# aanna0701/face-recognition-pytorch

Measured on AMD Instinct MI355X. Metric: train imgs/sec IR-50-layout ResNet50 + ArcFace/PartialFC head, 112x112, higher is better.
Workload: dtype bf16

## Files before the change

### face-recognition-pytorch_amd/frhip/csrc/igemm_nt.h

```cpp
#pragma once
#include "common.h"

namespace frhip {

struct NtGeom {
    int H, W, C;
    int Ho, Wo;
    int R, S, stride, pad;
    int mode;
    int M, Nout, Ktot;
    int ksteps, ksteps_per_split;
    uint32_t a_bytes, b_bytes;
    int par_a, par_b, hc, wc, par_r0, par_s0;
};

struct OutMap {
    int hc, wc, ho, wo, a, b;
    __device__ __forceinline__ long long row(int m) const {
        if (wc == 0) return m;
        const int per = hc * wc;
        const int img = m / per, rem = m - img * per;
        const int i = rem / wc, j = rem - i * wc;
        return ((long long)img * ho + 2 * i + a) * wo + 2 * j + b;
    }
};

constexpr int NT_ROWB = 128;

struct EpiBnRed {
    const void* y;
    const float* mean;
    const float* invstd;
    const float* mscale;
    const float* mshift;
    int res_h, res_w;
    OutMap map;
    const float* bias;
    void* act;
    int gelu_bwd;
    const float* aff_scale;
    const float* aff_shift;
    int aff_relu;
    const float* rowkeep;
    int rows_per;
    float keep_scale;
};

template <typename T, int WM, int WN, int MT = 4>
struct NtTile {
    static constexpr int WAVES = WM * WN, THREADS = 64 * WAVES;
    static constexpr int WROWS = MT * 16;
    static constexpr int BM = WM * WROWS, BN = WN * 64;
    static constexpr int BKE = NT_ROWB / (int)sizeof(T);
    static constexpr int STAGE_BYTES = (BM + BN) * NT_ROWB;
    static constexpr int A_PIECES = BM / 8 / WAVES, B_PIECES = BN / 8 / WAVES;
    static_assert(A_PIECES * 8 * WAVES == BM && B_PIECES * 8 * WAVES == BN, "tile rows must split evenly over the waves");
    template <typename TS> static constexpr int stage_pitch() { return 64 * (int)sizeof(TS) + 16; }
    template <typename TS> static constexpr int lds_bytes() {
        return (2 * STAGE_BYTES > WAVES * WROWS * stage_pitch<TS>()) ? 2 * STAGE_BYTES : WAVES * WROWS * stage_pitch<TS>();
    }
};

template <int NPIECE>
struct RowSet {
    int pixbase[NPIECE];
    int hb[NPIECE], wb[NPIECE];
};

template <typename T, int WM, int WN, int MT = 4>
struct NtMainloop {
    typedef NtTile<T, WM, WN, MT> Tile;
    typedef typename Mma<T>::Frag Frag;
    static constexpr int BM = Tile::BM, BN = Tile::BN, BKE = Tile::BKE;

    f32x4_t acc[4][MT];

    __device__ __forceinline__ void run(const NtGeom& g, const void* __restrict__ a_ptr,
                                        const void* __restrict__ b_ptr, char* smem,
                                        int mtile, int ntile, int ks_begin, int ks_end) {
        const int lane = lane_id();
        const int wave = wave_id();
        const int wm = wave / WN, wn = wave % WN;
#pragma unroll
        for (int i = 0; i < 4; ++i)
#pragma unroll
            for (int j = 0; j < MT; ++j) acc[i][j] = f32x4_t{0.f, 0.f, 0.f, 0.f};
        if (ks_begin >= ks_end) return;

        const __amdgpu_buffer_rsrc_t ra = make_rsrc(a_ptr, g.a_bytes);
        const __amdgpu_buffer_rsrc_t rb = make_rsrc(b_ptr, g.b_bytes);

        const int sub = lane >> 3;
        const uint32_t chunk_bytes = (uint32_t)(((lane & 7) ^ sub) * 16);
        RowSet<Tile::A_PIECES> ar;
        const int rowlen = g.par_a >= 0 ? g.wc : g.Wo;
        const int HoWo = g.par_a >= 0 ? g.hc * g.wc : g.Ho * g.Wo;
#pragma unroll
        for (int j = 0; j < Tile::A_PIECES; ++j) {
            const int row = (wave * Tile::A_PIECES + j) * 8 + sub;
            const int m = mtile * BM + row;
            if (m < g.M) {
                const int n = m / HoWo, rem = m - n * HoWo;
                int ho = rem / rowlen, wo = rem - ho * rowlen;
                if (g.par_a >= 0) { ho = 2 * ho + g.par_a; wo = 2 * wo + g.par_b; }
                ar.pixbase[j] = n * g.H * g.W;
                if (g.mode == 0) { ar.hb[j] = ho * g.stride - g.pad; ar.wb[j] = wo * g.stride - g.pad; }
                else             { ar.hb[j] = ho + g.pad;            ar.wb[j] = wo + g.pad; }
            } else {
                ar.pixbase[j] = -1; ar.hb[j] = 0; ar.wb[j] = 0;
            }
        }
        uint32_t brow_off[Tile::B_PIECES];
#pragma unroll
        for (int j = 0; j < Tile::B_PIECES; ++j) {
            const int row = (wave * Tile::B_PIECES + j) * 8 + sub;
            const int n = ntile * BN + row;
            brow_off[j] = (n < g.Nout) ? (uint32_t)n * (uint32_t)g.Ktot * (uint32_t)sizeof(T) + chunk_bytes
                                       : OOB_OFFSET;
        }

        const int cchunks = g.C / BKE;
        int tap = ks_begin / cchunks;
        int c0 = (ks_begin - tap * cchunks) * BKE;
        int fr = tap / g.S, fs = tap - fr * g.S;
        const int tstep = g.par_a >= 0 ? 2 : 1, fs0 = g.par_a >= 0 ? g.par_s0 : 0;
        if (g.par_a >= 0) {
            const int ns = (g.S - g.par_s0 + 1) >> 1;
            const int ir = tap / ns, is = tap - ir * ns;
            fr = g.par_r0 + 2 * ir; fs = g.par_s0 + 2 * is;
            tap = fr * g.S + fs;
        }

        auto stage = [&](int buf) {
            char* sa = smem + buf * Tile::STAGE_BYTES;
            char* sb = sa + BM * NT_ROWB;
#pragma unroll
            for (int j = 0; j < Tile::A_PIECES; ++j) {
                int hi, wi; bool ok = ar.pixbase[j] >= 0;
                if (g.mode == 0) {
                    hi = ar.hb[j] + fr; wi = ar.wb[j] + fs;
                } else {
                    const int th = ar.hb[j] - fr, tw = ar.wb[j] - fs;
                    ok = ok && th >= 0 && tw >= 0;
                    if (g.stride == 2) { ok = ok && !((th | tw) & 1); hi = th >> 1; wi = tw >> 1; }
                    else { hi = th; wi = tw; }
                }
                ok = ok && (unsigned)hi < (unsigned)g.H && (unsigned)wi < (unsigned)g.W;
                const uint32_t off = ok ? (uint32_t)((ar.pixbase[j] + hi * g.W + wi) * g.C + c0) * (uint32_t)sizeof(T) + chunk_bytes
                                        : OOB_OFFSET;
                glds16(ra, sa + (wave * Tile::A_PIECES + j) * 1024, off);
            }
            const uint32_t kb = (uint32_t)(tap * g.C + c0) * (uint32_t)sizeof(T);
#pragma unroll
            for (int j = 0; j < Tile::B_PIECES; ++j) {
                const uint32_t off = brow_off[j] == OOB_OFFSET ? OOB_OFFSET : brow_off[j] + kb;
                glds16(rb, sb + (wave * Tile::B_PIECES + j) * 1024, off);
// ... 37 lines not shown
        compute(cur);
    }

    __device__ __forceinline__ char* stage_half(char* smem, int h) {
        constexpr int P = Tile::template stage_pitch<bf16_t>();
        const int lane = lane_id();
        const int fi = lane & 15, fg = lane >> 4;
        char* mine = smem + wave_id() * Tile::WROWS * P;
        __syncthreads();
#pragma unroll
        for (int nt = 0; nt < 4; ++nt)
#pragma unroll
            for (int mt = 0; mt < 4; ++mt) {
                bf16x4_t v;
#pragma unroll
                for (int e = 0; e < 4; ++e) v[e] = (bf16_t)(h ? acc[nt][(MT > 4 ? 4 : 0) + mt][e] : acc[nt][mt][e]);
                *reinterpret_cast<bf16x4_t*>(mine + (mt * 16 + fi) * P + (nt * 16 + 4 * fg) * 2) = v;
            }
        __syncthreads();
        return mine;
    }

    template <typename TS>
    __device__ __forceinline__ char* stage_out(char* smem) {
        constexpr int P = Tile::template stage_pitch<TS>();
        const int lane = lane_id();
        const int fi = lane & 15, fg = lane >> 4;
        char* mine = smem + wave_id() * Tile::WROWS * P;
        __syncthreads();
#pragma unroll
        for (int nt = 0; nt < 4; ++nt)
#pragma unroll
            for (int mt = 0; mt < MT; ++mt) {
                char* p = mine + (mt * 16 + fi) * P + (nt * 16 + 4 * fg) * (int)sizeof(TS);
                if constexpr (sizeof(TS) == 4) {
                    *reinterpret_cast<f32x4_t*>(p) = acc[nt][mt];
                } else {
                    bf16x4_t v;
#pragma unroll
                    for (int e = 0; e < 4; ++e) v[e] = (bf16_t)acc[nt][mt][e];
                    *reinterpret_cast<bf16x4_t*>(p) = v;
                }
            }
        __syncthreads();
        return mine;
    }
};

template <typename T, int WROWS>
struct EpiOperands {
    static constexpr int EPV = 16 / (int)sizeof(T), LPR = 64 / EPV, RPI = 64 / LPR, ITERS = WROWS / RPI;
    static constexpr bool PRE = ITERS <= 8;
    Vec16<T> rv[PRE ? ITERS : 1], yv[PRE ? ITERS : 1];
    const T* r; const T* y;
    int M, Nout, m0, n, rsub;
    int res_h, res_w;
    OutMap map;
    uint32_t voff, vstep;
    static constexpr bool CAN_FAST = PRE && sizeof(T) == 2;
    __device__ __forceinline__ long long res_index(int m) const {
        if (res_w == 0) return (long long)m * Nout + n;
        const int hw = res_h * res_w;
        const int img = m / hw, rem = m - img * hw;
        const int h = rem / res_w, w = rem - h * res_w;
        if ((h | w) & 1) return -1;
        const int hc = (res_h + 1) >> 1, wc = (res_w + 1) >> 1;
        return ((long long)(img * hc + (h >> 1)) * wc + (w >> 1)) * Nout + n;
    }
    __device__ __forceinline__ void fetch(const void* __restrict__ res, const void* __restrict__ ybn, int M_, int Nout_,
                                          int m0_, int n0, int res_h_ = 0, int res_w_ = 0, const OutMap* map_ = nullptr) {
        const int lane = lane_id();
        M = M_; Nout = Nout_; m0 = m0_; res_h = res_h_; res_w = res_w_;
        if (map_) map = *map_; else map.wc = 0;
        n = n0 + (lane % LPR) * EPV; rsub = lane / LPR;
        r = reinterpret_cast<const T*>(res);
        y = reinterpret_cast<const T*>(ybn);
        if constexpr (PRE) {
#pragma unroll
            for (int it = 0; it < ITERS; ++it) {
                const int m = m0 + it * RPI + rsub;
                const bool ok = m < M && n < Nout;
                const size_t idx = (size_t)map.row(m) * Nout + n;
                if (r && ok) {
                    const long long ri = res_index((int)map.row(m));
                    if (ri >= 0) rv[it] = *reinterpret_cast<const Vec16<T>*>(r + ri);
                    else {
#pragma unroll
                        for (int e = 0; e < EPV; ++e) rv[it].set(e, 0.f);
                    }
                }
                if (y && ok) yv[it] = *reinterpret_cast<const Vec16<T>*>(y + idx);
            }
        }
    }
    __device__ __forceinline__ void fetch_fast(const void* __restrict__ res, const void* __restrict__ ybn, int M_, int Nout_,
                                               int m0_, int n0) {
        static_assert(CAN_FAST, "lean epilogue: bf16 tiles of at most 64 rows per wave");
        const int lane = lane_id();
        M = M_; Nout = Nout_; m0 = m0_; res_h = 0; res_w = 0; map.wc = 0;
        n = n0 + (lane % LPR) * EPV; rsub = lane / LPR;
        r = reinterpret_cast<const T*>(res);
        y = reinterpret_cast<const T*>(ybn);
        const uint32_t bytes = (uint32_t)M * (uint32_t)Nout * (uint32_t)sizeof(T);
        voff = ((uint32_t)(m0 + rsub) * (uint32_t)Nout + (uint32_t)n) * (uint32_t)sizeof(T);
        vstep = (uint32_t)RPI * (uint32_t)Nout * (uint32_t)sizeof(T);
        if (r) {
            const __amdgpu_buffer_rsrc_t rr = make_rsrc(res, bytes);
#pragma unroll
            for (int it = 0; it < ITERS; ++it)
                rv[it].v = __builtin_bit_cast(decltype(rv[it].v), __builtin_amdgcn_raw_buffer_load_b128(rr, voff, it * vstep, 0));
        }
        if (y) {
            const __amdgpu_buffer_rsrc_t ry = make_rsrc(ybn, bytes);
#pragma unroll
            for (int it = 0; it < ITERS; ++it)
                yv[it].v = __builtin_bit_cast(decltype(yv[it].v), __builtin_amdgcn_raw_buffer_load_b128(ry, voff, it * vstep, 0));
        }
    }
    __device__ __forceinline__ Vec16<T> res_row(int it) const {
        if constexpr (PRE) return rv[it];
        else {
            const long long ri = res_index((int)map.row(m0 + it * RPI + rsub));
            Vec16<T> z;
#pragma unroll
            for (int e = 0; e < EPV; ++e) z.set(e, 0.f);
            return ri >= 0 ? *reinterpret_cast<const Vec16<T>*>(r + ri) : z;
        }
    }
    __device__ __forceinline__ Vec16<T> y_row(int it) const {
        if constexpr (PRE) return yv[it];
        else return *reinterpret_cast<const Vec16<T>*>(y + (size_t)map.row(m0 + it * RPI + rsub) * Nout + n);
    }
};

inline bool epi_lean_ok(bool bf16, long long M, int Nout, int bm, int bn, const EpiBnRed& br) {
    return bf16 && M % bm == 0 && Nout % bn == 0 && br.map.wc == 0 && br.res_w == 0 && !br.bias && !br.act && !br.gelu_bwd &&
           M * Nout * 2 < 0x7fffffffLL;
}

template <typename T> __device__ __forceinline__ void epi_store_row(T* p, const Vec16<T>& v) {
    __builtin_nontemporal_store(v.v, reinterpret_cast<decltype(v.v)*>(p));
}

__device__ __forceinline__ bf16x8_t epi_tr_frag(const char* tile, int P, int r0, int c0, int lane) {
    const int g = lane >> 4, j = lane & 15, q = j >> 2, p = j & 3;
    const char* pa = tile + (r0 + 8 * g + q) * P + (c0 + 4 * p) * 2;
    typedef __attribute__((address_space(3))) i16x4_t* lds_p;
    const i16x4_t lo = __builtin_amdgcn_ds_read_tr16_b64_v4i16((lds_p)LDS_ADDR(pa));
    const i16x4_t hi = __builtin_amdgcn_ds_read_tr16_b64_v4i16((lds_p)LDS_ADDR(pa + 4 * P));
    typedef __attribute__((ext_vector_type(8))) short i16x8_t;
    return __builtin_bit_cast(bf16x8_t, (i16x8_t)__builtin_shufflevector(lo, hi, 0, 1, 2, 3, 4, 5, 6, 7));
}
template <int WROWS>
__device__ __forceinline__ void epi_mfma_sums(const char* tx, const char* tz, int P, f32x4_t (&S)[4], f32x4_t (&G)[4]) {
    const int lane = lane_id();
    bf16x8_t ones;
#pragma unroll
    for (int e = 0; e < 8; ++e) ones[e] = (bf16_t)1.0f;
#pragma unroll
    for (int cb = 0; cb < 4; ++cb) { S[cb] = f32x4_t{0.f, 0.f, 0.f, 0.f}; G[cb] = f32x4_t{0.f, 0.f, 0.f, 0.f}; }
#pragma unroll
    for (int ks = 0; ks < WROWS / 32; ++ks)
#pragma unroll
        for (int cb = 0; cb < 4; ++cb) {
            const bf16x8_t fx = epi_tr_frag(tx, P, 32 * ks, 16 * cb, lane);
            const bf16x8_t fz = (tz == tx) ? fx : epi_tr_frag(tz, P, 32 * ks, 16 * cb, lane);
            S[cb] = __builtin_amdgcn_mfma_f32_16x16x32_bf16(ones, fx, S[cb], 0, 0, 0);
            G[cb] = __builtin_amdgcn_mfma_f32_16x16x32_bf16(fx, fz, G[cb], 0, 0, 0);
        }
}
__device__ __forceinline__ float epi_diag(const f32x4_t& g, int lane) {
    const int e = lane & 3;
    return e == 0 ? g[0] : (e == 1 ? g[1] : (e == 2 ? g[2] : g[3]));
}
template <int WM, int WN, int THREADS, int BN>
__device__ __forceinline__ void epi_stats_tail_mfma(const float (&a1)[4], const float (&a2)[4], char* smem, int Nout,
                                                    float* __restrict__ stats, int mtile, int ntile) {
    const int lane = lane_id(), wave = wave_id();
    const int g = lane >> 4, j = lane & 15;
    __syncthreads();
    float* red = reinterpret_cast<float*>(smem);
    if ((j >> 2) == g) {
#pragma unroll
        for (int cb = 0; cb < 4; ++cb) {
// ... 187 lines not shown
                for (int e = 0; e < EPV; ++e) {
                    ga.set(e, gelu_value<T>(v.get(e)));
                }
                const __amdgpu_buffer_rsrc_t ra = make_rsrc(br.act, bytes);
                store_b128<0>(__builtin_bit_cast(u32x4_t, ga.v), ra, voff, it * vstep);
            }
            if (rewrite) *reinterpret_cast<Vec16<T>*>(src + it * RPI * P) = v;
        }
    }
    if (stats) {
        f32x4_t S[4], G[4];
        epi_mfma_sums<WROWS>(mine, mine, P, S, G);
        float a1[4], a2[4];
#pragma unroll
        for (int cb = 0; cb < 4; ++cb) { a1[cb] = S[cb][0]; a2[cb] = epi_diag(G[cb], lane); }
        epi_stats_tail_mfma<WM, WN, THREADS, BN>(a1, a2, smem, Nout, stats, mtile, ntile);
    }
}

inline bool nt_lean_ok(bool bf16, long long M, int Nout, const EpiBnRed& br, const float* stats) {
    return bf16 && M % 256 == 0 && Nout % 256 == 0 && br.map.wc == 0 && br.res_w == 0 && !br.aff_scale &&
           !(stats && br.y && !br.gelu_bwd && (br.bias || br.act)) && M * Nout * 2 < 0x7fffffffLL;
}

template <typename T, int WM, int WN, int WROWS, int THREADS, int BN>
__device__ __forceinline__ void nt_epilogue_store(const char* mine, int P, char* smem, int M, int Nout,
                                                  void* __restrict__ out, bool has_res, float* __restrict__ stats,
                                                  const EpiBnRed& br, const EpiOperands<T, WROWS>& ops, int mtile,
                                                  int ntile, int m0, int n0) {
    constexpr int EPV = 16 / (int)sizeof(T);
    constexpr int LPR = 64 / EPV;
    constexpr int RPI = 64 / LPR;
    const int lane = lane_id(), wave = wave_id();
    const int chunk = lane % LPR, rsub = lane / LPR;
    const int n = n0 + chunk * EPV;
    float s1[EPV], s2[EPV];
#pragma unroll
    for (int e = 0; e < EPV; ++e) { s1[e] = 0.f; s2[e] = 0.f; }
    T* o = reinterpret_cast<T*>(out);
    if (stats && br.y && !br.gelu_bwd) {
        float mu[EPV], is[EPV], ms[EPV], mb[EPV];
#pragma unroll
        for (int e = 0; e < EPV; ++e) {
            const bool ok = n + e < Nout;
            mu[e] = ok ? br.mean[n + e] : 0.f; is[e] = ok ? br.invstd[n + e] : 0.f;
            ms[e] = (ok && br.mscale) ? br.mscale[n + e] : 0.f; mb[e] = (ok && br.mscale) ? br.mshift[n + e] : 1.f;
        }
#pragma unroll
        for (int it = 0; it < WROWS / RPI; ++it) {
            const int row = it * RPI + rsub;
            const int m = m0 + row;
            Vec16<T> v = *reinterpret_cast<const Vec16<T>*>(mine + row * P + chunk * 16);
            if (m < M && n < Nout) {
                if (has_res) {
                    const Vec16<T> rr = ops.res_row(it);
#pragma unroll
                    for (int e = 0; e < EPV; ++e) v.set(e, v.get(e) + rr.get(e));
                }
                epi_store_row(o + (size_t)br.map.row(m) * Nout + n, v);
                const Vec16<T> yr = ops.y_row(it);
                const float kf = br.rowkeep ? (br.rowkeep[m / br.rows_per] != 0.f ? br.keep_scale : 0.f) : 1.f;
#pragma unroll
                for (int e = 0; e < EPV; ++e) {
                    const float yy = yr.get(e);
                    const float d = (yy * ms[e] + mb[e] > 0.f) ? v.get(e) * kf : 0.f;
                    s1[e] += d; s2[e] += d * (yy - mu[e]) * is[e];
                }
            }
        }
    } else {
        float bb[EPV];
#pragma unroll
        for (int e = 0; e < EPV; ++e) bb[e] = (br.bias && n + e < Nout) ? br.bias[n + e] : 0.f;
        T* ao = reinterpret_cast<T*>(br.act);
#pragma unroll
        for (int it = 0; it < WROWS / RPI; ++it) {
            const int row = it * RPI + rsub;
            const int m = m0 + row;
            Vec16<T> v = *reinterpret_cast<const Vec16<T>*>(mine + row * P + chunk * 16);
            if (m < M && n < Nout) {
                if (has_res) {
                    const Vec16<T> rr = ops.res_row(it);
#pragma unroll
                    for (int e = 0; e < EPV; ++e) v.set(e, v.get(e) + rr.get(e));
                }
                if (br.bias) {
#pragma unroll
                    for (int e = 0; e < EPV; ++e) v.set(e, v.get(e) + bb[e]);
                }
                if (br.gelu_bwd) {
                    const Vec16<T> hv = ops.y_row(it);
#pragma unroll
                    for (int e = 0; e < EPV; ++e) {
                        v.set(e, v.get(e) * gelu_slope<T>(hv.get(e)));
                    }
                }
                const size_t orow = (size_t)br.map.row(m);
                epi_store_row(o + orow * Nout + n, v);
                if (ao) {
                    Vec16<T> ga;
#pragma unroll
                    for (int e = 0; e < EPV; ++e) {
                        ga.set(e, gelu_value<T>(v.get(e)));
                    }
                    *reinterpret_cast<Vec16<T>*>(ao + orow * Nout + n) = ga;
                }
            }
#pragma unroll
            for (int e = 0; e < EPV; ++e) { const float x = v.get(e); s1[e] += x; s2[e] += x * x; }
        }
    }
    if (stats) {
#pragma unroll
        for (int e = 0; e < EPV; ++e) {
            if constexpr (LPR <= 8) { s1[e] = lane_sum_bit3(s1[e]); s2[e] = lane_sum_bit3(s2[e]); }
            if constexpr (LPR <= 16) { s1[e] = lane_sum_bit4(s1[e]); s2[e] = lane_sum_bit4(s2[e]); }
            s1[e] = lane_sum_bit5(s1[e]); s2[e] = lane_sum_bit5(s2[e]);
        }
        static_assert(LPR == 8 || LPR == 16, "lanes per 64-channel row");
        __syncthreads();
        float* red = reinterpret_cast<float*>(smem);
        if (lane < LPR) {
#pragma unroll
            for (int e = 0; e < EPV; ++e) {
                red[(wave * 2 + 0) * 64 + chunk * EPV + e] = s1[e];
                red[(wave * 2 + 1) * 64 + chunk * EPV + e] = s2[e];
            }
        }
        __syncthreads();
        for (int t = threadIdx.x; t < WN * 2 * 64; t += THREADS) {
            const int c = t & 63, st = (t >> 6) & 1, w_n = t >> 7;
            float a = 0.f;
#pragma unroll
            for (int w_m = 0; w_m < WM; ++w_m) a += red[((w_m * WN + w_n) * 2 + st) * 64 + c];
            const int nn = ntile * BN + w_n * 64 + c;
            if (nn < Nout) stats[((size_t)mtile * 2 + st) * Nout + nn] = a;
        }
    }
}

}
```

### face-recognition-pytorch_amd/frhip/csrc/igemm_nt.hip

```cpp
#include "igemm_nt.h"
#include "frhip.h"

namespace frhip {

bool halo_applicable(int dtype, int h, int w, int c, int k, int r, int s, int stride, int pad);
int halo_stat_rows(int dtype, int m, int w, int c, int k, int sign);
bool halo_xf_applicable(int dtype, int h, int w, int c, int k, int r, int s, int stride, int pad);
bool halo_lean_applies(int dtype, int n, int h, int w, int c, int k, int sign);
int halo_run(int dtype, const void* a, const void* b, void* out, const void* res, float* stats, const EpiBnRed& br,
             int n, int h, int w, int c, int k, int sign, hipStream_t stream, const float* xf_scale = nullptr,
             const float* xf_shift = nullptr, void* xf_out = nullptr);

enum { EPI_STORE = 0, EPI_ATOMIC = 1, EPI_SLAB = 2, EPI_LEAN = 3 };
extern int g_epi_lean;

template <typename T, int WM, int WN, int MT, int EPI>
__device__ __forceinline__ void nt_tile(const NtGeom& g, const void* __restrict__ a, const void* __restrict__ b, void* __restrict__ out,
                                        const void* __restrict__ res, float* __restrict__ stats, const EpiBnRed& br, int ntiles,
                                        uint32_t t, uint32_t total, char* smem) {
    typedef NtTile<T, WM, WN, MT> Tile;
    constexpr int WROWS = Tile::WROWS, THREADS = Tile::THREADS;
    const uint32_t lin = xcd_remap(t, total);
    const int ntile = (int)(lin % (uint32_t)ntiles), mtile = (int)(lin / (uint32_t)ntiles);
    const int ks_begin = blockIdx.y * g.ksteps_per_split;
// ... 34 lines not shown
        constexpr int P = Tile::template stage_pitch<float>();
        const char* mine = ml.template stage_out<float>(smem);
        float* o = reinterpret_cast<float*>(out);
        const int n = n0 + lane;
        if constexpr (EPI == EPI_SLAB) o += (size_t)blockIdx.y * g.M * g.Nout;
        for (int row = 0; row < WROWS; ++row) {
            const int m = m0 + row;
            if (m < g.M && n < g.Nout) {
                const float v = *reinterpret_cast<const float*>(mine + row * P + lane * 4);
                if constexpr (EPI == EPI_SLAB) o[(size_t)m * g.Nout + n] = v;
                else atomicAdd(o + (size_t)m * g.Nout + n, v);
            }
        }
    }
}

template <typename T, int WM, int WN, int MT, int EPI>
__global__ __launch_bounds__(64 * WM * WN, (WM * WN) / 4) void nt_kernel(NtGeom g, const void* __restrict__ a,
                                                           const void* __restrict__ b, void* __restrict__ out,
                                                           const void* __restrict__ res, float* __restrict__ stats,
                                                           EpiBnRed br, int mtiles, int ntiles) {
    extern __shared__ __attribute__((aligned(16))) char smem[];
    const uint32_t total = (uint32_t)(mtiles * ntiles);
    if constexpr (EPI == EPI_LEAN) {
        for (uint32_t t = blockIdx.x; t < total; t += gridDim.x) {
            nt_tile<T, WM, WN, MT, EPI>(g, a, b, out, res, stats, br, ntiles, t, total, smem);
            if (t + gridDim.x < total) {
                asm volatile("s_waitcnt lgkmcnt(0)" ::: "memory");
                __builtin_amdgcn_s_barrier();
            }
        }
    } else {
        nt_tile<T, WM, WN, MT, EPI>(g, a, b, out, res, stats, br, ntiles, blockIdx.x, total, smem);
    }
}

template <typename T, int WM, int WN, int MT, int EPI>
static int nt_launch_cfg(const NtGeom& g, const void* a, const void* b, void* out, const void* res,
                         float* stats, const EpiBnRed& br, int splits, hipStream_t stream) {
    typedef NtTile<T, WM, WN, MT> Tile;
    const int mtiles = (g.M + Tile::BM - 1) / Tile::BM, ntiles = (g.Nout + Tile::BN - 1) / Tile::BN;
    const int lds = (EPI == EPI_STORE || EPI == EPI_LEAN) ? Tile::template lds_bytes<T>() : Tile::template lds_bytes<float>();
    auto kern = nt_kernel<T, WM, WN, MT, EPI>;
    if (set_dynamic_lds(reinterpret_cast<const void*>(kern), lds, "igemm_nt")) return FRHIP_ELAUNCH;
    dim3 grid(mtiles * ntiles, splits);
    if (EPI == EPI_LEAN) {
        const unsigned wgs = (unsigned)device_cu_count() & ~7u;
        if (wgs >= 8 && grid.x > wgs) grid.x = wgs;
    }
    hipLaunchKernelGGL(kern, grid, dim3(Tile::THREADS), lds, stream, g, a, b, out, res, stats, br, mtiles, ntiles);
    return check_launch("igemm_nt");
}

static int g_nt_tile = 0;

static int nt_pick_tile(int dtype, const NtGeom& g) {
    if (g_nt_tile) return (dtype != FRHIP_DT_BF16 && g_nt_tile >= 3) ? 1 : g_nt_tile;
    if ((g.Nout % 128) != 0 && g.Nout <= 256) return 2;
    if (dtype == FRHIP_DT_BF16 && (g.Nout % 256) == 0 && g.M >= 256 * 64) return 4;
    return 1;
}

static const EpiBnRed NO_BNRED = {nullptr, nullptr, nullptr, nullptr, nullptr, 0, 0, {0, 0, 0, 0, 0, 0}, nullptr, nullptr, 0};

static int nt_dispatch(int dtype, const NtGeom& g, const void* a, const void* b, void* out, const void* res,
                       float* stats, const EpiBnRed& br, int splits, bool atomic, hipStream_t stream) {
    const int tile = nt_pick_tile(dtype, g);
#define NT_GO(T, WM, WN, MT)                                                                              \
    return atomic ? nt_launch_cfg<T, WM, WN, MT, EPI_ATOMIC>(g, a, b, out, res, stats, br, splits, stream)     \
                  : nt_launch_cfg<T, WM, WN, MT, EPI_STORE>(g, a, b, out, res, stats, br, splits, stream)
    if (dtype == FRHIP_DT_BF16 && (tile == 3 || tile == 4)) {
        if (tile == 4 && !atomic && splits == 1 && g_epi_lean && nt_lean_ok(true, g.M, g.Nout, br, stats))
            return nt_launch_cfg<bf16_t, 2, 4, 8, EPI_LEAN>(g, a, b, out, res, stats, br, splits, stream);
        if (tile == 4 && !atomic) return nt_launch_cfg<bf16_t, 2, 4, 8, EPI_STORE>(g, a, b, out, res, stats, br, splits, stream);
        NT_GO(bf16_t, 4, 2, 4);
    }
    return by_dtype(dtype, "igemm_nt", [&](auto t) {
        typedef decltype(t) T;
        if (tile == 2) NT_GO(T, 4, 1, 4);
        NT_GO(T, 2, 2, 4);
    });
#undef NT_GO
}

static int esize(int dtype) { return dtype == FRHIP_DT_BF16 ? 2 : 4; }

static int fill_geom(NtGeom& g, int dtype, int n, int h, int w, int c, int ho, int wo, int k, int r, int s,
                     int stride, int pad, int mode, const char* who) {
    const int bke = NT_ROWB / esize(dtype);
    if (n <= 0 || h <= 0 || w <= 0 || c <= 0 || k <= 0 || (c % bke) != 0 || (k % 8) != 0 || (stride != 1 && stride != 2)) {
        set_error("%s: unsupported shape n=%d h=%d w=%d c=%d k=%d stride=%d (c must be a multiple of %d, k of 8)",
                  who, n, h, w, c, k, stride, bke);
        return FRHIP_EINVAL;
    }
    const long long a_bytes = 1LL * n * h * w * c * esize(dtype), b_bytes = 1LL * k * r * s * c * esize(dtype);
    if (a_bytes > 0x7fffffffLL || b_bytes > 0x7fffffffLL || 1LL * n * ho * wo > 0x7fffffffLL) {
        set_error("%s: tensor exceeds the 2 GiB buffer-addressing window", who);
        return FRHIP_EINVAL;
    }
    g.H = h; g.W = w; g.C = c; g.Ho = ho; g.Wo = wo; g.R = r; g.S = s; g.stride = stride; g.pad = pad; g.mode = mode;
    g.M = n * ho * wo; g.Nout = k; g.Ktot = r * s * c;
    g.ksteps = r * s * (c / bke); g.ksteps_per_split = g.ksteps;
    g.a_bytes = (uint32_t)a_bytes; g.b_bytes = (uint32_t)b_bytes;
    g.par_a = -1; g.par_b = -1; g.hc = 0; g.wc = 0; g.par_r0 = 0; g.par_s0 = 0;
    return FRHIP_OK;
}

static bool dgrad_by_parity(const NtGeom& g) { return g.mode == 1 && g.stride == 2 && g.R == 3 && g.S == 3 && g.pad == 1; }

static int nt_block_rows(int dtype, const NtGeom& g) {
    static const int bm_of[5] = {128, 128, 256, 256, 256};
    return bm_of[nt_pick_tile(dtype, g)];
}

static int parity_class(const NtGeom& g, int dtype, int a, int b, NtGeom& gc, OutMap& map) {
    gc = g;
    gc.par_a = a; gc.par_b = b;
    gc.hc = (g.Ho - a + 1) / 2; gc.wc = (g.Wo - b + 1) / 2;
    gc.par_r0 = (a + g.pad) & 1; gc.par_s0 = (b + g.pad) & 1;
    const int nr = (g.R - gc.par_r0 + 1) / 2, ns = (g.S - gc.par_s0 + 1) / 2;
    const int n_img = g.M / (g.Ho * g.Wo);
    gc.M = n_img * gc.hc * gc.wc;
    gc.ksteps = nr * ns * (g.C / (NT_ROWB / (dtype == FRHIP_DT_BF16 ? 2 : 4)));
    gc.ksteps_per_split = gc.ksteps;
    map.hc = gc.hc; map.wc = gc.wc; map.ho = g.Ho; map.wo = g.Wo; map.a = a; map.b = b;
    return gc.M;
}

}

using namespace frhip;

extern "C" int frhip_nt_block_m(int nout) {
    return ((nout % 128) == 0 || nout > 256) ? 128 : 256;
}
extern "C" int frhip_conv_stat_rows(int dtype, int m, int k, int h, int w, int c, int r, int s, int stride, int pad) {
    if (halo_applicable(dtype, h, w, c, k, r, s, stride, pad)) return halo_stat_rows(dtype, m, w, c, k, +1);
    NtGeom g; g.M = m; g.Nout = k;
    static const int bm_of[5] = {128, 128, 256, 256, 256};
    const int bm = bm_of[nt_pick_tile(dtype, g)];
    return (m + bm - 1) / bm;
}
extern "C" int frhip_set_nt_tile(int tile) { const int old = g_nt_tile; g_nt_tile = tile; return old; }

extern "C" int frhip_conv_fwd(int dtype, const void* x, const void* w, void* y, float* stats_partial,
                              int n, int h, int wd, int c, int k, int r, int s, int stride, int pad,
                              hipStream_t stream) {
    if (const int rc = by_dtype(dtype, "frhip_conv_fwd", [](auto) { return FRHIP_OK; })) return rc;
    NtGeom g;
    const int ho = (h + 2 * pad - r) / stride + 1, wo = (wd + 2 * pad - s) / stride + 1;
    int rc = fill_geom(g, dtype, n, h, wd, c, ho, wo, k, r, s, stride, pad, 0, "frhip_conv_fwd");
    if (rc) return rc;
    if (halo_applicable(dtype, h, wd, c, k, r, s, stride, pad))
        return halo_run(dtype, x, w, y, nullptr, stats_partial, NO_BNRED, n, h, wd, c, k, +1, stream);
    return nt_dispatch(dtype, g, x, w, y, nullptr, stats_partial, NO_BNRED, 1, false, stream);
}

extern "C" int frhip_conv_fwd_affine(int dtype, const void* x, const void* w, void* y, const float* scale, const float* shift, int relu,
                                     const void* residual, int n, int h, int wd, int c, int k, int r, int s, int stride, int pad,
                                     hipStream_t stream) {
    if (const int rc = by_dtype(dtype, "frhip_conv_fwd_affine", [](auto) { return FRHIP_OK; })) return rc;
    if (!scale || !shift) { set_error("frhip_conv_fwd_affine: scale and shift are required"); return FRHIP_EINVAL; }
    NtGeom g;
    const int ho = (h + 2 * pad - r) / stride + 1, wo = (wd + 2 * pad - s) / stride + 1;
    int rc = fill_geom(g, dtype, n, h, wd, c, ho, wo, k, r, s, stride, pad, 0, "frhip_conv_fwd_affine");
    if (rc) return rc;
    if (halo_applicable(dtype, h, wd, c, k, r, s, stride, pad) && halo_lean_applies(dtype, n, h, wd, c, k, +1)) {
        EpiBnRed br = NO_BNRED;
        br.aff_scale = scale; br.aff_shift = shift; br.aff_relu = relu;
        return halo_run(dtype, x, w, y, residual, nullptr, br, n, h, wd, c, k, +1, stream);
    }
    rc = frhip_conv_fwd(dtype, x, w, y, nullptr, n, h, wd, c, k, r, s, stride, pad, stream);
    if (rc) return rc;
    return frhip_bn_apply(dtype, y, scale, shift, residual, nullptr, nullptr, relu, y, n * ho * wo, k, stream);
}

extern "C" int frhip_conv_bnrelu_fusable(int dtype, int h, int wd, int c, int k, int r, int s, int stride, int pad) {
    return halo_xf_applicable(dtype, h, wd, c, k, r, s, stride, pad) ? 1 : 0;
}

extern "C" int frhip_conv_fwd_bnrelu(int dtype, const void* x, const float* in_scale, const float* in_shift, const void* w, void* y,
                                     float* stats_partial, void* act_out, int n, int h, int wd, int c, int k, int r, int s, int stride,
                                     int pad, hipStream_t stream) {
    if (const int rc = by_dtype(dtype, "frhip_conv_fwd_bnrelu", [](auto) { return FRHIP_OK; })) return rc;
    if (!in_scale || !in_shift || !halo_xf_applicable(dtype, h, wd, c, k, r, s, stride, pad)) {
        set_error("frhip_conv_fwd_bnrelu: not fusable for this shape (ask frhip_conv_bnrelu_fusable first)");
        return FRHIP_EINVAL;
    }
    return halo_run(dtype, x, w, y, nullptr, stats_partial, NO_BNRED, n, h, wd, c, k, +1, stream, in_scale, in_shift, act_out);
}

static int dgrad_run(int dtype, const void* dy, const void* wt, void* dx, const void* residual, float* stats,
                     const EpiBnRed& br, int n, int h, int wd, int c, int k, int r, int s, int stride, int pad,
                     hipStream_t stream, const char* who) {
    NtGeom g;
    const int ho = (h + 2 * pad - r) / stride + 1, wo = (wd + 2 * pad - s) / stride + 1;
    int rc = fill_geom(g, dtype, n, ho, wo, k, h, wd, c, r, s, stride, pad, 1, who);
    if (rc) return rc;
    if (halo_applicable(dtype, h, wd, k, c, r, s, stride, pad))
        return halo_run(dtype, dy, wt, dx, residual, stats, br, n, h, wd, k, c, -1, stream);
    if (dgrad_by_parity(g)) {
        float* st = stats;
        for (int cls = 0; cls < 4; ++cls) {
            NtGeom gc; EpiBnRed bc = br;
            if (parity_class(g, dtype, cls >> 1, cls & 1, gc, bc.map) == 0) continue;
            rc = nt_dispatch(dtype, gc, dy, wt, dx, residual, st, bc, 1, false, stream);
            if (rc) return rc;
            if (st) st += (size_t)((gc.M + nt_block_rows(dtype, gc) - 1) / nt_block_rows(dtype, gc)) * 2 * gc.Nout;
        }
        return FRHIP_OK;
    }
    return nt_dispatch(dtype, g, dy, wt, dx, residual, stats, br, 1, false, stream);
}

extern "C" int frhip_conv_dgrad(int dtype, const void* dy, const void* wt, void* dx, const void* residual,
                                int n, int h, int wd, int c, int k, int r, int s, int stride, int pad,
                                hipStream_t stream) {
    if (const int rc = by_dtype(dtype, "frhip_conv_dgrad", [](auto) { return FRHIP_OK; })) return rc;
    return dgrad_run(dtype, dy, wt, dx, residual, nullptr, NO_BNRED, n, h, wd, c, k, r, s, stride, pad, stream, "frhip_conv_dgrad");
}

extern "C" int frhip_dgrad_stat_rows(int dtype, int n, int h, int wd, int c, int k, int r, int s, int stride, int pad) {
    const int m = n * h * wd;
    if (halo_applicable(dtype, h, wd, k, c, r, s, stride, pad)) return halo_stat_rows(dtype, m, wd, k, c, -1);
    NtGeom g; g.M = m; g.Nout = c;
    g.mode = 1; g.stride = stride; g.R = r; g.S = s; g.pad = pad; g.Ho = h; g.Wo = wd; g.C = k;
    if (dgrad_by_parity(g)) {
        int rows = 0;
        for (int cls = 0; cls < 4; ++cls) {
            NtGeom gc; OutMap map;
            const int mc = parity_class(g, dtype, cls >> 1, cls & 1, gc, map);
            rows += (mc + nt_block_rows(dtype, gc) - 1) / nt_block_rows(dtype, gc);
        }
        return rows;
    }
    const int bm = nt_block_rows(dtype, g);
    return (m + bm - 1) / bm;
}

extern "C" int frhip_conv_dgrad_fused(int dtype, const void* dy, const void* wt, void* dx, const void* residual,
                                      int residual_stride, const void* y_bn, const float* mean, const float* invstd,
                                      const float* mask_scale, const float* mask_shift, float* stats_partial, int n, int h,
                                      int wd, int c, int k, int r, int s, int stride, int pad, hipStream_t stream) {
    if (const int rc = by_dtype(dtype, "frhip_conv_dgrad_fused", [](auto) { return FRHIP_OK; })) return rc;
    if (residual_stride != 1 && residual_stride != 2) { set_error("frhip_conv_dgrad_fused: residual_stride must be 1 or 2"); return FRHIP_EINVAL; }
    if (y_bn && (!mean || !invstd || !stats_partial || (mask_scale && !mask_shift))) {
        set_error("frhip_conv_dgrad_fused: y_bn needs mean, invstd and stats_partial");
        return FRHIP_EINVAL;
    }
    EpiBnRed br = {y_bn, mean, invstd, mask_scale, mask_shift, 0, 0, {0, 0, 0, 0, 0, 0}, nullptr, nullptr, 0};
    if (residual && residual_stride == 2) { br.res_h = h; br.res_w = wd; }
    return dgrad_run(dtype, dy, wt, dx, residual, y_bn ? stats_partial : nullptr, br, n, h, wd, c, k, r, s, stride, pad, stream,
                     "frhip_conv_dgrad_fused");
}

extern "C" int frhip_conv_dgrad_fused_rs(int dtype, const void* dy, const void* wt, void* dx, const void* residual,
                                         int residual_stride, const void* y_bn, const float* mean, const float* invstd,
                                         const float* mask_scale, const float* mask_shift, const float* rowscale, int rows_per,
                                         float keep_scale, float* stats_partial, int n, int h, int wd, int c, int k, int r, int s,
                                         int stride, int pad, hipStream_t stream) {
    if (const int rc = by_dtype(dtype, "frhip_conv_dgrad_fused_rs", [](auto) { return FRHIP_OK; })) return rc;
    if (residual_stride != 1 && residual_stride != 2) { set_error("frhip_conv_dgrad_fused_rs: residual_stride must be 1 or 2"); return FRHIP_EINVAL; }
    if (!y_bn || !mean || !invstd || !stats_partial || (mask_scale && !mask_shift) || !rowscale || rows_per <= 0 ||
        (long long)n * h * wd % rows_per != 0) {
        set_error("frhip_conv_dgrad_fused_rs: y_bn, mean, invstd, stats_partial, rowscale and a rows_per that divides the rows are required");
        return FRHIP_EINVAL;
    }
    EpiBnRed br = {y_bn, mean, invstd, mask_scale, mask_shift, 0, 0, {0, 0, 0, 0, 0, 0}, nullptr, nullptr, 0};
    br.rowkeep = rowscale; br.rows_per = rows_per; br.keep_scale = keep_scale;
    if (residual && residual_stride == 2) { br.res_h = h; br.res_w = wd; }
    return dgrad_run(dtype, dy, wt, dx, residual, stats_partial, br, n, h, wd, c, k, r, s, stride, pad, stream, "frhip_conv_dgrad_fused_rs");
}

extern "C" int frhip_conv_dgrad_bnred(int dtype, const void* dy, const void* wt, void* dx, const void* residual,
                                      const void* y_bn, const float* mean, const float* invstd, const float* mask_scale,
                                      const float* mask_shift, float* stats_partial, int n, int h, int wd, int c, int k,
                                      int r, int s, int stride, int pad, hipStream_t stream) {
    if (const int rc = by_dtype(dtype, "frhip_conv_dgrad_bnred", [](auto) { return FRHIP_OK; })) return rc;
    if (!y_bn || !mean || !invstd || !stats_partial || (mask_scale && !mask_shift)) {
        set_error("frhip_conv_dgrad_bnred: y_bn, mean, invstd and stats_partial are required");
        return FRHIP_EINVAL;
    }
    return frhip_conv_dgrad_fused(dtype, dy, wt, dx, residual, 1, y_bn, mean, invstd, mask_scale, mask_shift, stats_partial,
                                  n, h, wd, c, k, r, s, stride, pad, stream);
}

extern "C" int frhip_linear_fwd(int dtype, const void* a, const void* w, const float* bias, void* out, void* act_out,
                                float* stats_partial, int m, int n, int k, hipStream_t stream) {
    if (const int rc = by_dtype(dtype, "frhip_linear_fwd", [](auto) { return FRHIP_OK; })) return rc;
    NtGeom g;
    int rc = fill_geom(g, dtype, m, 1, 1, k, 1, 1, n, 1, 1, 1, 0, 0, "frhip_linear_fwd");
    if (rc) return rc;
    EpiBnRed br = NO_BNRED;
    br.bias = bias; br.act = act_out;
    return nt_dispatch(dtype, g, a, w, out, nullptr, stats_partial, br, 1, false, stream);
}

extern "C" int frhip_linear_dgrad_gelu(int dtype, const void* dy, const void* wt, const void* pre, void* dx,
                                       float* stats_partial, int m, int n, int k, hipStream_t stream) {
    if (const int rc = by_dtype(dtype, "frhip_linear_dgrad_gelu", [](auto) { return FRHIP_OK; })) return rc;
    if (!pre) { set_error("frhip_linear_dgrad_gelu: the saved pre-activation is required"); return FRHIP_EINVAL; }
    NtGeom g;
    int rc = fill_geom(g, dtype, m, 1, 1, k, 1, 1, n, 1, 1, 1, 0, 0, "frhip_linear_dgrad_gelu");
    if (rc) return rc;
    EpiBnRed br = NO_BNRED;
    br.y = pre; br.gelu_bwd = 1;
    return nt_dispatch(dtype, g, dy, wt, dx, nullptr, stats_partial, br, 1, false, stream);
}

namespace frhip {
__global__ __launch_bounds__(256) void nt_slab_reduce_kernel(const float* __restrict__ slabs, int splits, size_t elems,
                                                             const float* __restrict__ bias, int n, float* __restrict__ out) {
    const size_t i = ((size_t)blockIdx.x * 256 + threadIdx.x) * 4;
    if (i >= elems) return;
    f32x4_t acc = *reinterpret_cast<const f32x4_t*>(slabs + i);
    for (int s = 1; s < splits; ++s) acc += *reinterpret_cast<const f32x4_t*>(slabs + (size_t)s * elems + i);
    if (bias) acc += *reinterpret_cast<const f32x4_t*>(bias + (i % (size_t)n));
    *reinterpret_cast<f32x4_t*>(out + i) = acc;
}
}

extern "C" int frhip_gemm_nt_splitk(int dtype, const void* a, const void* b, const float* bias, float* out, int m, int n,
                                    int k, int splits, float* slabs, size_t slab_bytes, hipStream_t stream) {
// ... 31 lines not shown
```

Baseline: 22470.

## Merge strided dgrad parity classes into one launch and use fast division for row maps

```diff
diff --git a/face-recognition-pytorch_amd/frhip/csrc/igemm_nt.h b/face-recognition-pytorch_amd/frhip/csrc/igemm_nt.h
--- a/face-recognition-pytorch_amd/frhip/csrc/igemm_nt.h
+++ b/face-recognition-pytorch_amd/frhip/csrc/igemm_nt.h
@@ -12,17 +12,15 @@
     int ksteps, ksteps_per_split;
     uint32_t a_bytes, b_bytes;
     int par_a, par_b, hc, wc, par_r0, par_s0;
+    FastDiv d_img = {0, 0, 0}, d_row = {0, 0, 0};
 };
+
+__device__ __forceinline__ int row_div(int n, const FastDiv& f, int d) { return f.d ? (int)fdiv((uint32_t)n, f) : n / d; }
 
 struct OutMap {
     int hc, wc, ho, wo, a, b;
-    __device__ __forceinline__ long long row(int m) const {
-        if (wc == 0) return m;
-        const int per = hc * wc;
-        const int img = m / per, rem = m - img * per;
-        const int i = rem / wc, j = rem - i * wc;
-        return ((long long)img * ho + 2 * i + a) * wo + 2 * j + b;
-    }
+    FastDiv d_per, d_wc;
+    FastDiv d_rhw, d_rw;
 };
 
 constexpr int NT_ROWB = 128;
@@ -95,13 +93,14 @@
         RowSet<Tile::A_PIECES> ar;
         const int rowlen = g.par_a >= 0 ? g.wc : g.Wo;
         const int HoWo = g.par_a >= 0 ? g.hc * g.wc : g.Ho * g.Wo;
+        const FastDiv d_img = g.d_img, d_row = g.d_row;
 #pragma unroll
         for (int j = 0; j < Tile::A_PIECES; ++j) {
             const int row = (wave * Tile::A_PIECES + j) * 8 + sub;
             const int m = mtile * BM + row;
             if (m < g.M) {
-                const int n = m / HoWo, rem = m - n * HoWo;
-                int ho = rem / rowlen, wo = rem - ho * rowlen;
+                const int n = row_div(m, d_img, HoWo), rem = m - n * HoWo;
+                int ho = row_div(rem, d_row, rowlen), wo = rem - ho * rowlen;
                 if (g.par_a >= 0) { ho = 2 * ho + g.par_a; wo = 2 * wo + g.par_b; }
                 ar.pixbase[j] = n * g.H * g.W;
                 if (g.mode == 0) { ar.hb[j] = ho * g.stride - g.pad; ar.wb[j] = wo * g.stride - g.pad; }
@@ -245,20 +244,30 @@
     static constexpr int EPV = 16 / (int)sizeof(T), LPR = 64 / EPV, RPI = 64 / LPR, ITERS = WROWS / RPI;
     static constexpr bool PRE = ITERS <= 8;
     Vec16<T> rv[PRE ? ITERS : 1], yv[PRE ? ITERS : 1];
+    int orow[PRE ? ITERS : 1];
     const T* r; const T* y;
     int M, Nout, m0, n, rsub;
     int res_h, res_w;
     OutMap map;
     uint32_t voff, vstep;
     static constexpr bool CAN_FAST = PRE && sizeof(T) == 2;
-    __device__ __forceinline__ long long res_index(int m) const {
-        if (res_w == 0) return (long long)m * Nout + n;
-        const int hw = res_h * res_w;
-        const int img = m / hw, rem = m - img * hw;
-        const int h = rem / res_w, w = rem - h * res_w;
-        if ((h | w) & 1) return -1;
-        const int hc = (res_h + 1) >> 1, wc = (res_w + 1) >> 1;
-        return ((long long)(img * hc + (h >> 1)) * wc + (w >> 1)) * Nout + n;
+    __device__ __forceinline__ void locate(int m, int& o, int& rr) const {
+        if (map.wc == 0 && res_w == 0) { o = m; rr = m; return; }
+        int img, h, w;
+        if (map.wc != 0) {
+            img = (int)fdiv((uint32_t)m, map.d_per);
+            const int rem = m - img * (map.hc * map.wc);
+            const int i = (int)fdiv((uint32_t)rem, map.d_wc), j = rem - i * map.wc;
+            h = 2 * i + map.a; w = 2 * j + map.b;
+            o = (img * map.ho + h) * map.wo + w;
+        } else {
+            img = (int)fdiv((uint32_t)m, map.d_rhw);
+            const int rem = m - img * (res_h * res_w);
+            h = (int)fdiv((uint32_t)rem, map.d_rw); w = rem - h * res_w;
+            o = m;
+        }
+        if (res_w == 0) rr = o;
+        else rr = ((h | w) & 1) ? -1 : (img * ((res_h + 1) >> 1) + (h >> 1)) * ((res_w + 1) >> 1) + (w >> 1);
     }
     __device__ __forceinline__ void fetch(const void* __restrict__ res, const void* __restrict__ ybn, int M_, int Nout_,
                                           int m0_, int n0, int res_h_ = 0, int res_w_ = 0, const OutMap* map_ = nullptr) {
@@ -273,16 +282,16 @@
             for (int it = 0; it < ITERS; ++it) {
                 const int m = m0 + it * RPI + rsub;
                 const bool ok = m < M && n < Nout;
-                const size_t idx = (size_t)map.row(m) * Nout + n;
+                int rr;
+                locate(m, orow[it], rr);
                 if (r && ok) {
-                    const long long ri = res_index((int)map.row(m));
-                    if (ri >= 0) rv[it] = *reinterpret_cast<const Vec16<T>*>(r + ri);
+                    if (rr >= 0) rv[it] = *reinterpret_cast<const Vec16<T>*>(r + (size_t)rr * Nout + n);
                     else {
 #pragma unroll
                         for (int e = 0; e < EPV; ++e) rv[it].set(e, 0.f);
                     }
                 }
-                if (y && ok) yv[it] = *reinterpret_cast<const Vec16<T>*>(y + idx);
+                if (y && ok) yv[it] = *reinterpret_cast<const Vec16<T>*>(y + (size_t)orow[it] * Nout + n);
             }
         }
     }
@@ -310,19 +319,22 @@
                 yv[it].v = __builtin_bit_cast(decltype(yv[it].v), __builtin_amdgcn_raw_buffer_load_b128(ry, voff, it * vstep, 0));
         }
     }
-    __device__ __forceinline__ Vec16<T> res_row(int it) const {
+    __device__ __forceinline__ void row_at(int it, int& o, int& rr) const {
+        if constexpr (PRE) { o = orow[it]; rr = 0; }
+        else locate(m0 + it * RPI + rsub, o, rr);
+    }
+    __device__ __forceinline__ Vec16<T> res_row(int it, int rr) const {
         if constexpr (PRE) return rv[it];
         else {
-            const long long ri = res_index((int)map.row(m0 + it * RPI + rsub));
             Vec16<T> z;
 #pragma unroll
             for (int e = 0; e < EPV; ++e) z.set(e, 0.f);
-            return ri >= 0 ? *reinterpret_cast<const Vec16<T>*>(r + ri) : z;
-        }
-    }
-    __device__ __forceinline__ Vec16<T> y_row(int it) const {
+            return rr >= 0 ? *reinterpret_cast<const Vec16<T>*>(r + (size_t)rr * Nout + n) : z;
+        }
+    }
+    __device__ __forceinline__ Vec16<T> y_row(int it, int o) const {
         if constexpr (PRE) return yv[it];
-        else return *reinterpret_cast<const Vec16<T>*>(y + (size_t)map.row(m0 + it * RPI + rsub) * Nout + n);
+        else return *reinterpret_cast<const Vec16<T>*>(y + (size_t)o * Nout + n);
     }
 };
 
@@ -616,13 +628,15 @@
             const int m = m0 + row;
             Vec16<T> v = *reinterpret_cast<const Vec16<T>*>(mine + row * P + chunk * 16);
             if (m < M && n < Nout) {
+                int orow, rrow;
+                ops.row_at(it, orow, rrow);
                 if (has_res) {
-                    const Vec16<T> rr = ops.res_row(it);
+                    const Vec16<T> rr = ops.res_row(it, rrow);
 #pragma unroll
                     for (int e = 0; e < EPV; ++e) v.set(e, v.get(e) + rr.get(e));
                 }
-                epi_store_row(o + (size_t)br.map.row(m) * Nout + n, v);
-                const Vec16<T> yr = ops.y_row(it);
+                epi_store_row(o + (size_t)orow * Nout + n, v);
+                const Vec16<T> yr = ops.y_row(it, orow);
                 const float kf = br.rowkeep ? (br.rowkeep[m / br.rows_per] != 0.f ? br.keep_scale : 0.f) : 1.f;
 #pragma unroll
                 for (int e = 0; e < EPV; ++e) {
@@ -643,8 +657,10 @@
             const int m = m0 + row;
             Vec16<T> v = *reinterpret_cast<const Vec16<T>*>(mine + row * P + chunk * 16);
             if (m < M && n < Nout) {
+                int orw, rrow;
+                ops.row_at(it, orw, rrow);
                 if (has_res) {
-                    const Vec16<T> rr = ops.res_row(it);
+                    const Vec16<T> rr = ops.res_row(it, rrow);
 #pragma unroll
                     for (int e = 0; e < EPV; ++e) v.set(e, v.get(e) + rr.get(e));
                 }
@@ -653,13 +669,13 @@
                     for (int e = 0; e < EPV; ++e) v.set(e, v.get(e) + bb[e]);
                 }
                 if (br.gelu_bwd) {
-                    const Vec16<T> hv = ops.y_row(it);
+                    const Vec16<T> hv = ops.y_row(it, orw);
 #pragma unroll
                     for (int e = 0; e < EPV; ++e) {
                         v.set(e, v.get(e) * gelu_slope<T>(hv.get(e)));
                     }
                 }
-                const size_t orow = (size_t)br.map.row(m);
+                const size_t orow = (size_t)orw;
                 epi_store_row(o + orow * Nout + n, v);
                 if (ao) {
                     Vec16<T> ga;
diff --git a/face-recognition-pytorch_amd/frhip/csrc/igemm_nt.hip b/face-recognition-pytorch_amd/frhip/csrc/igemm_nt.hip
--- a/face-recognition-pytorch_amd/frhip/csrc/igemm_nt.hip
+++ b/face-recognition-pytorch_amd/frhip/csrc/igemm_nt.hip
@@ -110,6 +110,59 @@
     return check_launch("igemm_nt");
 }
 
+struct ParityClass {
+    int par_a, par_b, hc, wc, par_r0, par_s0, M, ksteps;
+    FastDiv d_img, d_row;
+    OutMap map;
+    uint32_t tile0, tiles, stat_row0;
+};
+struct ParityTable { ParityClass cls[4]; };
+
+template <typename T, int WM, int WN, int MT>
+__global__ __launch_bounds__(64 * WM * WN, (WM * WN) / 4) void nt_parity_kernel(NtGeom g, ParityTable tab, const void* __restrict__ a,
+                                                                  const void* __restrict__ b, void* __restrict__ out,
+                                                                  const void* __restrict__ res, float* __restrict__ stats,
+                                                                  EpiBnRed br, int ntiles) {
+    extern __shared__ __attribute__((aligned(16))) char smem[];
+    ParityClass pc = tab.cls[0];
+#pragma unroll
+    for (int i = 1; i < 4; ++i)
+        if (blockIdx.x >= tab.cls[i].tile0) pc = tab.cls[i];
+    g.par_a = pc.par_a; g.par_b = pc.par_b; g.hc = pc.hc; g.wc = pc.wc; g.par_r0 = pc.par_r0; g.par_s0 = pc.par_s0;
+    g.M = pc.M; g.ksteps = pc.ksteps; g.ksteps_per_split = pc.ksteps; g.d_img = pc.d_img; g.d_row = pc.d_row;
+    br.map = pc.map;
+    if (stats) stats += (size_t)pc.stat_row0 * 2 * g.Nout;
+    nt_tile<T, WM, WN, MT, EPI_STORE>(g, a, b, out, res, stats, br, ntiles, blockIdx.x - pc.tile0, pc.tiles, smem);
+}
+
+template <typename T, int WM, int WN, int MT>
+static int nt_parity_launch(const NtGeom& g, const NtGeom (&gc)[4], const OutMap (&map)[4], const void* a, const void* b, void* out,
+                            const void* res, float* stats, const EpiBnRed& br, hipStream_t stream) {
+    typedef NtTile<T, WM, WN, MT> Tile;
+    const int ntiles = (g.Nout + Tile::BN - 1) / Tile::BN;
+    ParityTable tab;
+    uint32_t stat_row0[4], row = 0;
+    for (int cls = 0; cls < 4; ++cls) { stat_row0[cls] = row; row += (uint32_t)((gc[cls].M + Tile::BM - 1) / Tile::BM); }
+    long long total = 0;
+    int slot = 0;
+    for (int cls = 3; cls >= 0; --cls) {
+        if (gc[cls].M == 0) continue;
+        ParityClass& pc = tab.cls[slot++];
+        const NtGeom& c = gc[cls];
+        pc.par_a = c.par_a; pc.par_b = c.par_b; pc.hc = c.hc; pc.wc = c.wc; pc.par_r0 = c.par_r0; pc.par_s0 = c.par_s0;
+        pc.M = c.M; pc.ksteps = c.ksteps; pc.d_img = c.d_img; pc.d_row = c.d_row; pc.map = map[cls];
+        pc.tile0 = (uint32_t)total; pc.tiles = (uint32_t)((c.M + Tile::BM - 1) / Tile::BM) * (uint32_t)ntiles; pc.stat_row0 = stat_row0[cls];
+        total += pc.tiles;
+    }
+    for (; slot < 4; ++slot) { tab.cls[slot] = tab.cls[0]; tab.cls[slot].tile0 = 0xffffffffu; }
+    if (total > 0x7fffffffLL) { set_error("igemm_nt: too many tiles for one launch"); return FRHIP_EINVAL; }
+    const int lds = Tile::template lds_bytes<T>();
+    auto kern = nt_parity_kernel<T, WM, WN, MT>;
+    if (set_dynamic_lds(reinterpret_cast<const void*>(kern), lds, "igemm_nt")) return FRHIP_ELAUNCH;
+    hipLaunchKernelGGL(kern, dim3((unsigned)total), dim3(Tile::THREADS), lds, stream, g, tab, a, b, out, res, stats, br, ntiles);
+    return check_launch("igemm_nt");
+}
+
 static int g_nt_tile = 0;
 
 static int nt_pick_tile(int dtype, const NtGeom& g) {
@@ -161,6 +214,7 @@
     g.ksteps = r * s * (c / bke); g.ksteps_per_split = g.ksteps;
     g.a_bytes = (uint32_t)a_bytes; g.b_bytes = (uint32_t)b_bytes;
     g.par_a = -1; g.par_b = -1; g.hc = 0; g.wc = 0; g.par_r0 = 0; g.par_s0 = 0;
+    if (ho > 0 && wo > 0) { g.d_img = make_fastdiv((uint32_t)(ho * wo)); g.d_row = make_fastdiv((uint32_t)wo); }
     return FRHIP_OK;
 }
 
@@ -182,7 +236,30 @@
     gc.ksteps = nr * ns * (g.C / (NT_ROWB / (dtype == FRHIP_DT_BF16 ? 2 : 4)));
     gc.ksteps_per_split = gc.ksteps;
     map.hc = gc.hc; map.wc = gc.wc; map.ho = g.Ho; map.wo = g.Wo; map.a = a; map.b = b;
+    if (gc.M > 0) {
+        gc.d_img = map.d_per = make_fastdiv((uint32_t)(gc.hc * gc.wc));
+        gc.d_row = map.d_wc = make_fastdiv((uint32_t)gc.wc);
+    }
     return gc.M;
+}
+
+static int parity_classes(const NtGeom& g, int dtype, NtGeom (&gc)[4], OutMap (&map)[4]) {
+    for (int cls = 0; cls < 4; ++cls) parity_class(g, dtype, cls >> 1, cls & 1, gc[cls], map[cls]);
+    return nt_pick_tile(dtype, gc[0]);
+}
+
+static int nt_parity_dispatch(int dtype, const NtGeom& g, const void* a, const void* b, void* out, const void* res, float* stats,
+                              const EpiBnRed& br, hipStream_t stream) {
+    NtGeom gc[4]; OutMap map[4];
+    for (int cls = 0; cls < 4; ++cls) map[cls] = br.map;
+    const int tile = parity_classes(g, dtype, gc, map);
+    if (dtype == FRHIP_DT_BF16 && tile == 4) return nt_parity_launch<bf16_t, 2, 4, 8>(g, gc, map, a, b, out, res, stats, br, stream);
+    if (dtype == FRHIP_DT_BF16 && tile == 3) return nt_parity_launch<bf16_t, 4, 2, 4>(g, gc, map, a, b, out, res, stats, br, stream);
+    return by_dtype(dtype, "igemm_nt", [&](auto t) {
+        typedef decltype(t) T;
+        if (tile == 2) return nt_parity_launch<T, 4, 1, 4>(g, gc, map, a, b, out, res, stats, br, stream);
+        return nt_parity_launch<T, 2, 2, 4>(g, gc, map, a, b, out, res, stats, br, stream);
+    });
 }
 
 }
@@ -248,6 +325,11 @@
     return halo_run(dtype, x, w, y, nullptr, stats_partial, NO_BNRED, n, h, wd, c, k, +1, stream, in_scale, in_shift, act_out);
 }
 
+static void compact_residual(EpiBnRed& br, int h, int wd) {
+    br.res_h = h; br.res_w = wd;
+    if (h > 0 && wd > 0) { br.map.d_rhw = make_fastdiv((uint32_t)h * (uint32_t)wd); br.map.d_rw = make_fastdiv((uint32_t)wd); }
+}
+
 static int dgrad_run(int dtype, const void* dy, const void* wt, void* dx, const void* residual, float* stats,
                      const EpiBnRed& br, int n, int h, int wd, int c, int k, int r, int s, int stride, int pad,
                      hipStream_t stream, const char* who) {
@@ -257,17 +339,7 @@
     if (rc) return rc;
     if (halo_applicable(dtype, h, wd, k, c, r, s, stride, pad))
         return halo_run(dtype, dy, wt, dx, residual, stats, br, n, h, wd, k, c, -1, stream);
-    if (dgrad_by_parity(g)) {
-        float* st = stats;
-        for (int cls = 0; cls < 4; ++cls) {
-            NtGeom gc; EpiBnRed bc = br;
-            if (parity_class(g, dtype, cls >> 1, cls & 1, gc, bc.map) == 0) continue;
-            rc = nt_dispatch(dtype, gc, dy, wt, dx, residual, st, bc, 1, false, stream);
-            if (rc) return rc;
-            if (st) st += (size_t)((gc.M + nt_block_rows(dtype, gc) - 1) / nt_block_rows(dtype, gc)) * 2 * gc.Nout;
-        }
-        return FRHIP_OK;
-    }
+    if (dgrad_by_parity(g)) return nt_parity_dispatch(dtype, g, dy, wt, dx, residual, stats, br, stream);
     return nt_dispatch(dtype, g, dy, wt, dx, residual, stats, br, 1, false, stream);
 }
 
@@ -284,12 +356,11 @@
     NtGeom g; g.M = m; g.Nout = c;
     g.mode = 1; g.stride = stride; g.R = r; g.S = s; g.pad = pad; g.Ho = h; g.Wo = wd; g.C = k;
     if (dgrad_by_parity(g)) {
+        NtGeom gc[4]; OutMap map[4];
+        static const int bm_of[5] = {128, 128, 256, 256, 256};
+        const int bm = bm_of[parity_classes(g, dtype, gc, map)];
         int rows = 0;
-        for (int cls = 0; cls < 4; ++cls) {
-            NtGeom gc; OutMap map;
-            const int mc = parity_class(g, dtype, cls >> 1, cls & 1, gc, map);
-            rows += (mc + nt_block_rows(dtype, gc) - 1) / nt_block_rows(dtype, gc);
-        }
+        for (int cls = 0; cls < 4; ++cls) rows += (gc[cls].M + bm - 1) / bm;
         return rows;
     }
     const int bm = nt_block_rows(dtype, g);
@@ -307,7 +378,7 @@
         return FRHIP_EINVAL;
     }
     EpiBnRed br = {y_bn, mean, invstd, mask_scale, mask_shift, 0, 0, {0, 0, 0, 0, 0, 0}, nullptr, nullptr, 0};
-    if (residual && residual_stride == 2) { br.res_h = h; br.res_w = wd; }
+    if (residual && residual_stride == 2) compact_residual(br, h, wd);
     return dgrad_run(dtype, dy, wt, dx, residual, y_bn ? stats_partial : nullptr, br, n, h, wd, c, k, r, s, stride, pad, stream,
                      "frhip_conv_dgrad_fused");
 }
@@ -326,7 +397,7 @@
     }
     EpiBnRed br = {y_bn, mean, invstd, mask_scale, mask_shift, 0, 0, {0, 0, 0, 0, 0, 0}, nullptr, nullptr, 0};
     br.rowkeep = rowscale; br.rows_per = rows_per; br.keep_scale = keep_scale;
-    if (residual && residual_stride == 2) { br.res_h = h; br.res_w = wd; }
+    if (residual && residual_stride == 2) compact_residual(br, h, wd);
     return dgrad_run(dtype, dy, wt, dx, residual, stats_partial, br, n, h, wd, c, k, r, s, stride, pad, stream, "frhip_conv_dgrad_fused_rs");
 }
 
```

After: 22560, median of 6. About the same (+0.4%).
